# KhutornoyYaroslav/vcm-ts

Hardware: AMD Instinct MI355X
Metric: encoded frames/sec at 1920x1080 GOP-32 (higher is better)
Workload: dtype f32 (fp16x3 split-MFMA, fp32 accumulate)

## Files before the change

include/dcvc_hip.h:

```cpp
#ifndef DCVC_HIP_H
#define DCVC_HIP_H

#include <stdint.h>

#ifdef __cplusplus
extern "C" {
#endif

#define DCVC_OK 0
#define DCVC_E_ARG (-1)
#define DCVC_E_LAUNCH (-2)
#define DCVC_E_RANGE (-3)

#define DCVC_STATUS_ACT_SATURATED 1

#define DCVC_MAX_SEG 3

#define DCVC_PREC_FP32 0
#define DCVC_PREC_FP16X3 1

typedef struct {
    const float *ptr;
    int32_t C;
    int32_t cs;
} dcvc_seg;

typedef struct {
    dcvc_seg seg[DCVC_MAX_SEG];
    int32_t nseg;
    int32_t N, Hin, Win;
    int32_t in_act;
    float in_slope;
    const float *wpack;
    const float *bpack;
    int32_t ks;
    int32_t stride;
    int32_t Cout;
    int32_t Cout_pad;
    float *out;
    int32_t out_cs;
    int32_t out_act;
    float out_slope;
    int32_t pixel_shuffle;
    const float *res;
    int32_t res_cs;
    const float *res_gate;
    const float *res2;
    int32_t res2_cs;
    int32_t precision;
    int32_t *status;
    float *chan_partial;
    int32_t tile_row0;
    int32_t tile_rows;
    int32_t pair_taps;
} dcvc_conv_args;

int32_t dcvc_conv_tile_rows(int32_t ks, int32_t stride);

int32_t dcvc_conv_chan_partial_parts(int32_t ks, int32_t stride, int32_t Hout, int32_t Wout);
int dcvc_channel_mean_finish(const float *chan_partial, int32_t parts, int32_t row_stride, float *mean, int32_t N,
                             int32_t C, int32_t HW, void *stream);

int64_t dcvc_conv_pack_size(int32_t Cout, int32_t ks, int32_t nseg, const int32_t *seg_C, int32_t *cout_pad);

int dcvc_conv_pack_weights(const float *w, const float *b, int32_t Cout, int32_t ks, int32_t nseg,
                           const int32_t *seg_C, int32_t pixel_shuffle, int32_t precision, float *wpack,
                           float *bpack);

int64_t dcvc_conv_pack_size_paired(int32_t Cout, int32_t Cin, int32_t *cout_pad);
int dcvc_conv_pack_weights_paired(const float *w, const float *b, int32_t Cout, int32_t Cin, float *wpack, float *bpack);

int dcvc_conv2d(const dcvc_conv_args *a, void *stream);

int64_t dcvc_conv_small_pack_bytes(int32_t Cout, int32_t ks, int32_t nseg, const int32_t *seg_C);
int dcvc_conv_small_pack_weights(const float *w, const float *b, int32_t Cout, int32_t ks, int32_t nseg,
                                 const int32_t *seg_C, void *wpack, float *bpack);
int dcvc_conv2d_small(const dcvc_conv_args *a, void *stream);

int64_t dcvc_conv_k32_pack_bytes(int32_t Cout, int32_t ks, int32_t nseg, const int32_t *seg_C, int32_t *cout_pad);
int dcvc_conv_k32_pack_weights(const float *w, const float *b, int32_t Cout, int32_t ks, int32_t nseg,
                               const int32_t *seg_C, int32_t pixel_shuffle, void *wpack, float *bpack);
int dcvc_conv2d_k32(const dcvc_conv_args *a, void *stream);
int dcvc_conv_k32_set_waves(int32_t waves);

int dcvc_warp(const float *src, int32_t src_cs, const float *flow, int32_t flow_cs, float *out, int32_t out_cs,
              int32_t N, int32_t H, int32_t W, int32_t C, void *stream);
int dcvc_up2(const float *src, int32_t src_cs, float *out, int32_t out_cs, float *out2, int32_t out2_cs,
             int32_t N, int32_t H, int32_t W, int32_t C, float scale, void *stream);
int dcvc_down2(const float *src, int32_t src_cs, float *out, int32_t out_cs, int32_t N, int32_t H, int32_t W,
               int32_t C, float scale, int32_t avgpool_order, void *stream);
int dcvc_maxpool2(const float *src, int32_t src_cs, float *out, int32_t out_cs, int32_t N, int32_t H, int32_t W,
                  int32_t C, void *stream);
int dcvc_copy_channels(const float *src, int32_t src_cs, float *out, int32_t out_cs, int64_t npix, int32_t C,
                       void *stream);
int dcvc_nchw_to_nhwc(const float *src, float *out, int32_t out_cs, int32_t N, int32_t C, int32_t H, int32_t W,
                      void *stream);
int dcvc_nhwc_to_nchw(const float *src, int32_t src_cs, float *out, int32_t N, int32_t C, int32_t H, int32_t W,
                      int32_t clamp01, void *stream);

int dcvc_channel_mean(const float *src, int32_t src_cs, float *mean, float *scratch, int32_t N, int32_t HW,
                      int32_t C, void *stream);
int dcvc_se_gate(const float *mean, const float *w1, const float *w2, float *gate, int32_t N, int32_t C,
                 int32_t Cr, void *stream);

int dcvc_scale_channels(const float *src, int32_t src_cs, float *out, int32_t out_cs, const float *q_basic,
                        const float *q_scale, int32_t mode, int32_t N, int32_t HW, int32_t C, void *stream);
int dcvc_round_symbols(const float *z, int32_t z_cs, float *z_hat, int32_t zh_cs, int32_t *sym, int32_t N,
                       int32_t H, int32_t W, int32_t C, void *stream);
int dcvc_symbols_to_nhwc(const int32_t *sym, float *out, int32_t out_cs, int32_t N, int32_t H, int32_t W,
                         int32_t C, void *stream);

typedef struct {
    const float *y;
    int32_t y_cs;
    const float *fusion;
    int32_t fusion_cs;
    const float *spatial;
    int32_t spatial_cs;
    float *params;
    int32_t params_cs;
    float *y_hat;
    float *y_q;
    float *y_res;
    float *scales_hat;
    int32_t *sym;
    int32_t *idx;
    float *out;
    int32_t out_cs;
    const float *q_basic;
    const float *q_scale;
    int32_t N, H, W, C;
    int32_t step;
    const float *idx_edges;
    const float *forced_q;
} dcvc_dual_prior_args;

int dcvc_scale_indexes(const float *scales, int32_t *idx, int64_t n, const float *idx_edges, void *stream);

int dcvc_dual_prior_enc(const dcvc_dual_prior_args *a, void *stream);
int dcvc_dual_prior_dec_index(const dcvc_dual_prior_args *a, void *stream);
int dcvc_dual_prior_dec_apply(const dcvc_dual_prior_args *a, void *stream);

int dcvc_scale_bits(const float *y_q, const float *scales_hat, float *out, float *scratch, int32_t kind, int32_t N,
                    int64_t per_sample, void *stream);
int dcvc_factorized_bits(const float *z_hat, int32_t z_cs, const float *params, float *out, float *scratch, int32_t N,
                         int32_t HW, int32_t C, void *stream);
int dcvc_sq_err(const float *a, int32_t a_cs, const float *b, int32_t b_cs, float *out, float *scratch, int32_t N,
                int32_t HW, int32_t C, void *stream);

int32_t dcvc_cdf_table_cols(void);
int dcvc_build_scale_cdfs(const float *scales, int32_t n_scales, int32_t kind, int32_t *cdf, int32_t *sizes,
                          int32_t *offsets, void *stream);
int dcvc_build_factorized_cdfs(const float *params, int32_t C, int32_t *cdf, int32_t *sizes, int32_t *offsets, void *stream);

const char *dcvc_hip_version(void);

#ifdef __cplusplus
}
#endif
#endif
```

vcm_ts_amd/csrc/conv_mfma.hip:

```cpp
#include <hip/hip_runtime.h>
#include <stdint.h>
#include <stdlib.h>
#include <string.h>
#include <vector>

#include "dcvc_hip.h"
#include "kernel_common.h"

namespace {

constexpr int LDK = 20;


struct ConvK {
    const float *seg_ptr[DCVC_MAX_SEG];
    int seg_C[DCVC_MAX_SEG];
    int seg_cs[DCVC_MAX_SEG];
    int nseg;
    int Hin, Win, Hout, Wout;
    int in_act;
    float in_slope;
    const float *wpack;
    const float *bpack;
    int Cout, Cout_pad;
    float *out;
    int out_cs;
    int out_act;
    float out_slope;
    int ps;
    const float *res;
    int res_cs;
    const float *res_gate;
    const float *res2;
    int res2_cs;
    int vec_epi;
    int *status;
    float *chan_partial;
    int ntx;
    int ty0, nty;
    int band_rows;
};

inline long dev_env_long(const char *name, long dflt) {
    const char *dev = getenv("DCVC_DEV");
    if (!dev || strcmp(dev, "1") != 0) return dflt;
    const char *v = getenv(name);
    return v ? atol(v) : dflt;
}


template <int KS, int S, int RPW, int NT, bool SPLIT, bool PAIR = false>
__global__ __launch_bounds__(256, 2) void conv_mfma(const ConvK a) {
    static_assert(!PAIR || (KS == 7 && S == 1 && SPLIT), "tap pairing is built for the 7x7 split-fp16 layers");
    constexpr int BH = 4 * RPW, BW = 32, BN = 32 * NT;
    constexpr int PH = (BH - 1) * S + KS, PW = (BW - 1) * S + KS, PAD = KS / 2;
    constexpr int T = PAIR ? KS * 4 : KS * KS;
    constexpr int TPS = PAIR ? 4 : (KS == 3 && S == 1) ? 9 : KS;
    constexpr int NST = T / TPS;
    constexpr int EPI_LD = BN + 4;
    constexpr int LDS_MAIN = PH * PW * LDK + TPS * 4 * BN * 4, LDS_EPI = 4 * 32 * EPI_LD, LDS_RED = 4 * BN;
    __shared__ __attribute__((aligned(16))) float lds[LDS_MAIN > LDS_EPI + LDS_RED ? LDS_MAIN : LDS_EPI + LDS_RED];
    float *patch = lds;
    float *wl = lds + PH * PW * LDK;

    const int tid = threadIdx.x, lane = tid & 63, wave = tid >> 6;
    const int nbn = a.Cout_pad / BN;
    const int nb = blockIdx.x % nbn, tx = blockIdx.x / nbn;
    if (tx >= a.ntx) return;
    const int ty = blockIdx.y + a.ty0;
    const int x0 = tx * BW, y0 = ty * BH, n0 = nb * BN, img = blockIdx.z;

    f32x16 acc[RPW][NT];
#pragma unroll
    for (int m = 0; m < RPW; ++m)
#pragma unroll
        for (int n = 0; n < NT; ++n)
#pragma unroll
            for (int r = 0; r < 16; ++r) acc[m][n][r] = 0.f;

    const int a_base = ((wave * RPW * S) * PW + (lane & 31) * S) * LDK + (lane >> 5) * 4;
    const int b_base = ((lane >> 5) * BN + (lane & 31)) * 4;

    constexpr int NP = (PH * PW * 4 + 255) / 256, NW = (TPS * 4 * BN + 255) / 256;
    f32x4 rp[NP], rw[NW];
    struct Cursor {
        int s, c0, cg, st;
    };
    auto advance = [&](Cursor &k) {
        if (++k.st == NST) {
            k.st = 0;
            ++k.cg;
            k.c0 += MFMA_KC;
            if (k.c0 >= a.seg_C[k.s]) {
                ++k.s;
                k.c0 = 0;
            }
        }
    };
    int poff[NP];
    unsigned inpic = 0;
#pragma unroll
    for (int u = 0; u < NP; ++u) {
        const int i = tid + u * 256;
        const int p = i >> 2;
        const int py = p / PW, px = p - py * PW + (PAIR ? (i & 3) >> 1 : 0);
        const int gy = y0 * S - PAD + py, gx = x0 * S - PAD + px;
        const bool ok = i < PH * PW * 4 && gy >= 0 && gy < a.Hin && gx >= 0 && gx < a.Win;
        poff[u] = ok ? gy * a.Win + gx : 0;
        inpic |= (ok ? 1u : 0u) << u;
    }
    auto load_patch = [&](const Cursor &k) {
        const int C = a.seg_C[k.s], cs = a.seg_cs[k.s];
        const float *sp = a.seg_ptr[k.s] + (size_t)img * a.Hin * a.Win * cs;
        const int c = PAIR ? (tid & 1) * 4 : k.c0 + (tid & 3) * 4;
        const int cc = c < C ? c : 0;
#pragma unroll
        for (int u = 0; u < NP; ++u) rp[u] = *(const f32x4 *)(sp + (size_t)poff[u] * cs + cc);
    };
    auto store_patch = [&](const Cursor &k) {
        const int C = a.seg_C[k.s];
#pragma unroll
        for (int u = 0; u < NP; ++u) {
            const int i = tid + u * 256;
            if (i < PH * PW * 4) {
                const int c = PAIR ? (i & 1) * 4 : k.c0 + (i & 3) * 4;
                f32x4 v = ((inpic >> u) & 1u) && c < C ? rp[u] : (f32x4){0.f, 0.f, 0.f, 0.f};
                if (c + 3 >= C) {
                    if (c + 1 >= C) v[1] = 0.f;
                    if (c + 2 >= C) v[2] = 0.f;
                    v[3] = 0.f;
                }
                if (a.in_act) {
                    v[0] = act(v[0], a.in_slope);
                    v[1] = act(v[1], a.in_slope);
                    v[2] = act(v[2], a.in_slope);
                    v[3] = act(v[3], a.in_slope);
                }
                if (!SPLIT) {
                    *(f32x4 *)&patch[(i >> 2) * LDK + (i & 3) * 4] = v;
                } else {
                    f32x4 sv = v * ACT_SCALE;
#pragma unroll
                    for (int e = 0; e < 4; ++e) sv[e] = __builtin_amdgcn_fmed3f(sv[e], -F16_MAX, F16_MAX);
                    const f16x4 hi = __builtin_convertvector(sv, f16x4);
                    const f16x4 lo = __builtin_convertvector(sv - __builtin_convertvector(hi, f32x4), f16x4);
                    _Float16 *rec = (_Float16 *)&patch[(i >> 2) * LDK];
                    *(f16x4 *)&rec[(i & 3) * 4] = hi;
                    *(f16x4 *)&rec[16 + (i & 3) * 4] = lo;
                }
            }
        }
    };
    auto load_w = [&](const Cursor &k) {
        const float *wsrc = a.wpack + ((size_t)(k.cg * T + k.st * TPS) * 4) * a.Cout_pad * 4 + (size_t)n0 * 4;
#pragma unroll
        for (int u = 0; u < NW; ++u) {
            const int i = tid + u * 256;
            const int row = i / BN, col = i - row * BN;
            if (i < TPS * 4 * BN) rw[u] = *(const f32x4 *)(wsrc + ((size_t)row * a.Cout_pad + col) * 4);
        }
    };
    auto store_w = [&]() {
#pragma unroll
        for (int u = 0; u < NW; ++u) {
            const int i = tid + u * 256;
            if (i < TPS * 4 * BN) *(f32x4 *)&wl[i * 4] = rw[u];
        }
    };

    Cursor cur = {0, 0, 0, 0};
    load_patch(cur);
    load_w(cur);
    while (cur.s < a.nseg) {
        __syncthreads();
        if (cur.st == 0) store_patch(cur);
        store_w();
        __syncthreads();
        Cursor nxt = cur;
        advance(nxt);
        if (nxt.s < a.nseg) {
            if (nxt.st == 0) load_patch(nxt);
            load_w(nxt);
        }
        const int a_st = (TPS == T) ? 0 : cur.st * PW * LDK;
#pragma unroll
        for (int tt = 0; tt < TPS; ++tt) {
            const int ky = (TPS == T) ? tt / KS : 0, kx = PAIR ? 2 * tt : (TPS == T) ? tt % KS : tt;
            if (!SPLIT) {
#pragma unroll
                for (int k2 = 0; k2 < 2; ++k2) {
                    f32x4 af[RPW], bf[NT];
#pragma unroll
                    for (int m = 0; m < RPW; ++m)
                        af[m] = *(const f32x4 *)&patch[a_base + a_st + ((m * S + ky) * PW + kx) * LDK + k2 * 8];
#pragma unroll
                    for (int n = 0; n < NT; ++n)
                        bf[n] = *(const f32x4 *)&wl[b_base + ((tt * 4 + k2 * 2) * BN + n * 32) * 4];
#pragma unroll
                    for (int j = 0; j < 4; ++j)
#pragma unroll
                        for (int m = 0; m < RPW; ++m)
// ... 144 lines not shown
            int dy = 0, dx = 0, cf = ch;
            if (a.ps) {
                const int sub = ch / Cq;
                cf = ch - sub * Cq;
                dy = sub >> 1;
                dx = sub & 1;
            }
            const float gate = a.res_gate ? a.res_gate[(size_t)img * Cfin + cf] : 1.f;
            float rv[16], rv2[16];
#pragma unroll
            for (int r = 0; r < 16; ++r) {
                const int ox = x0 + (r & 3) + 8 * (r >> 2) + 4 * hh;
                const size_t pix = a.ps ? ((size_t)(img * Ho + 2 * oy + dy) * Wo + 2 * ox + dx)
                                        : ((size_t)(img * Ho + oy) * Wo + ox);
                rv[r] = (a.res && ox < a.Wout) ? a.res[pix * a.res_cs + cf] : 0.f;
                rv2[r] = (a.res2 && ox < a.Wout) ? a.res2[pix * a.res2_cs + cf] : 0.f;
            }
#pragma unroll
            for (int r = 0; r < 16; ++r) {
                const int ox = x0 + (r & 3) + 8 * (r >> 2) + 4 * hh;
                if (ox >= a.Wout) continue;
                float v = acc[m][n][r] * inv_scale + bias;
                if (a.out_act == 1) v = act(v, a.out_slope);
                else if (a.out_act == 2) v = fminf(fmaxf(v, 0.f), 1.f);
                const size_t pix = a.ps ? ((size_t)(img * Ho + 2 * oy + dy) * Wo + 2 * ox + dx)
                                        : ((size_t)(img * Ho + oy) * Wo + ox);
                if (a.out_act == 3) {
                    const float mk = rv2[r] > 0.f ? 1.f : a.out_slope;
                    v = a.res ? __builtin_fmaf(v, mk, rv[r]) : v * mk;
                } else {
                    if (a.res) v = a.res_gate ? __builtin_fmaf(rv[r], gate, v) : v + rv[r];
                    if (a.res2) v = rv2[r] + v;
                }
                if (a.status) vmax = fmaxf(vmax, fabsf(v));
                a.out[pix * a.out_cs + cf] = v;
            }
        }
    }
    if (a.status && !(vmax <= ACT_LIMIT)) atomicOr(a.status, DCVC_STATUS_ACT_SATURATED);
}


template <int KS, int S, int RPW, int NT, bool PAIR = false>
int launch(ConvK &k, int N, hipStream_t st, int precision) {
    constexpr int BH = 4 * RPW, BN = 32 * NT;
    k.ntx = (k.Wout + 31) / 32;
    static const bool xcd_pad = dev_env_long("DCVC_XCD_PAD", 0) != 0;
    unsigned gx = (unsigned)(k.ntx * (k.Cout_pad / BN));
    if (xcd_pad && gx >= 8) gx = (gx + 7) & ~7u;
    k.nty = (k.Hout + BH - 1) / BH;
    if (k.ty0 < 0 || k.ty0 >= k.nty) return DCVC_E_ARG;
    const int rows = k.band_rows > 0 ? (k.band_rows < k.nty - k.ty0 ? k.band_rows : k.nty - k.ty0) : k.nty;
    dim3 grid(gx, (unsigned)rows, (unsigned)N);
    if (PAIR)
        hipLaunchKernelGGL((conv_mfma<KS, S, RPW, NT, true, PAIR>), grid, dim3(256), 0, st, k);
    else if (precision == DCVC_PREC_FP16X3)
        hipLaunchKernelGGL((conv_mfma<KS, S, RPW, NT, true>), grid, dim3(256), 0, st, k);
    else
        hipLaunchKernelGGL((conv_mfma<KS, S, RPW, NT, false>), grid, dim3(256), 0, st, k);
    RET_LAUNCH();
}

}

extern "C" int64_t dcvc_conv_pack_size(int32_t Cout, int32_t ks, int32_t nseg, const int32_t *seg_C, int32_t *cout_pad) {
    if (Cout <= 0 || nseg <= 0 || nseg > DCVC_MAX_SEG || (ks != 1 && ks != 3 && ks != 7)) return DCVC_E_ARG;
    int chunks = 0;
    for (int s = 0; s < nseg; ++s) chunks += (seg_C[s] + MFMA_KC - 1) / MFMA_KC;
    const int cp = round_up(Cout, 32);
    if (cout_pad) *cout_pad = cp;
    return (int64_t)chunks * ks * ks * 4 * cp * 4;
}

extern "C" int dcvc_conv_pack_weights(const float *w, const float *b, int32_t Cout, int32_t ks, int32_t nseg,
                                      const int32_t *seg_C, int32_t pixel_shuffle, int32_t precision, float *wpack,
                                      float *bpack) {
    if (precision != DCVC_PREC_FP32 && precision != DCVC_PREC_FP16X3) return DCVC_E_ARG;
    int32_t cp = 0;
    const int64_t total = dcvc_conv_pack_size(Cout, ks, nseg, seg_C, &cp);
    if (total < 0 || (pixel_shuffle && (Cout & 3))) return DCVC_E_ARG;
    const int T = ks * ks;
    int Cin = 0;
    for (int s = 0; s < nseg; ++s) Cin += seg_C[s];
    memset(wpack, 0, (size_t)total * sizeof(float));
    memset(bpack, 0, (size_t)cp * sizeof(float));
    const int Cq = Cout / 4;
    _Float16 *base = (_Float16 *)wpack;
    int cg = 0, cin0 = 0;
    for (int s = 0; s < nseg; ++s) {
        for (int c0 = 0; c0 < seg_C[s]; c0 += MFMA_KC, ++cg) {
            for (int t = 0; t < T; ++t)
                for (int cc = 0; cc < MFMA_KC && c0 + cc < seg_C[s]; ++cc)
                    for (int n = 0; n < Cout; ++n) {
                        const int np = pixel_shuffle ? ps_packed_channel(n, Cq) : n;
                        const float v = w[((size_t)n * Cin + cin0 + c0 + cc) * T + t];
                        if (precision == DCVC_PREC_FP32) {
                            wpack[mfma_wpack_f32(cg, T, t, cc, cp, np)] = v;
                        } else {
                            float sv = v * WGT_SCALE;
                            sv = sv > F16_MAX ? F16_MAX : (sv < -F16_MAX ? -F16_MAX : sv);
                            const SplitF16 p = split_f16(sv);
                            base[mfma_wpack_f16(cg, T, t, cc, cp, np, 0)] = p.hi;
                            base[mfma_wpack_f16(cg, T, t, cc, cp, np, 1)] = p.lo;
                        }
                    }
        }
        cin0 += seg_C[s];
    }
    for (int n = 0; n < Cout; ++n) bpack[pixel_shuffle ? ps_packed_channel(n, Cq) : n] = b ? b[n] : 0.f;
    return DCVC_OK;
}

extern "C" int64_t dcvc_conv_pack_size_paired(int32_t Cout, int32_t Cin, int32_t *cout_pad) {
    if (Cout <= 0 || Cin <= 0 || Cin > 8) return DCVC_E_ARG;
    const int cp = round_up(Cout, 32);
    if (cout_pad) *cout_pad = cp;
    return (int64_t)7 * 4 * 4 * cp * 4;
}

extern "C" int dcvc_conv_pack_weights_paired(const float *w, const float *b, int32_t Cout, int32_t Cin, float *wpack, float *bpack) {
    int32_t cp = 0;
    const int64_t total = dcvc_conv_pack_size_paired(Cout, Cin, &cp);
    if (total < 0 || !w || !wpack || !bpack) return DCVC_E_ARG;
    memset(wpack, 0, (size_t)total * sizeof(float));
    memset(bpack, 0, (size_t)cp * sizeof(float));
    _Float16 *base = (_Float16 *)wpack;
    bool clamped = false;
    for (int ky = 0; ky < 7; ++ky)
        for (int kx = 0; kx < 7; ++kx) {
            const int step = ky * 4 + (kx >> 1), h = kx & 1;
            for (int c = 0; c < Cin; ++c)
                for (int n = 0; n < Cout; ++n) {
                    float sv = w[((size_t)n * Cin + c) * 49 + ky * 7 + kx] * WGT_SCALE;
                    if (!(fabsf(sv) <= F16_MAX)) { clamped = true; sv = sv > 0.f ? F16_MAX : -F16_MAX; }
                    const SplitF16 p = split_f16(sv);
                    base[mfma_wpack_f16(0, 28, step, 8 * h + c, cp, n, 0)] = p.hi;
                    base[mfma_wpack_f16(0, 28, step, 8 * h + c, cp, n, 1)] = p.lo;
                }
        }
    for (int n = 0; n < Cout; ++n) bpack[n] = b ? b[n] : 0.f;
    return clamped ? DCVC_E_RANGE : DCVC_OK;
}

static int tile_rows(int ks, int stride) { return stride == 2 ? 4 : 8; }

extern "C" int32_t dcvc_conv_tile_rows(int32_t ks, int32_t stride) { return tile_rows(ks, stride); }

extern "C" int32_t dcvc_conv_chan_partial_parts(int32_t ks, int32_t stride, int32_t Hout, int32_t Wout) {
    if (Hout <= 0 || Wout <= 0 || (stride != 1 && stride != 2)) return DCVC_E_ARG;
    const int bh = tile_rows(ks, stride);
    return ((Wout + 31) / 32) * ((Hout + bh - 1) / bh);
}

extern "C" int dcvc_conv2d(const dcvc_conv_args *a, void *stream) {
    if (!conv_args_ok(a)) return DCVC_E_ARG;
    if (a->stride != 1 && a->stride != 2) return DCVC_E_ARG;
    if (a->precision != DCVC_PREC_FP32 && a->precision != DCVC_PREC_FP16X3) return DCVC_E_ARG;
    if (a->Cout_pad % 32 || a->Cout > a->Cout_pad || (a->pixel_shuffle && (a->Cout & 3))) return DCVC_E_ARG;
    if (a->out_act < 0 || a->out_act > 3) return DCVC_E_ARG;
    if (a->out_act == 3 && (!a->res2 || a->res_gate || a->chan_partial || a->pixel_shuffle)) return DCVC_E_ARG;
    ConvK k;
    memset(&k, 0, sizeof(k));
    copy_conv_args_full(k, a);
    k.Hin = a->Hin;
    k.Win = a->Win;
    const int pad = a->ks / 2;
    k.Hout = (a->Hin + 2 * pad - a->ks) / a->stride + 1;
    k.Wout = (a->Win + 2 * pad - a->ks) / a->stride + 1;
    k.vec_epi = vec_epilogue_ok(a);
    if (a->chan_partial && (!k.vec_epi || a->pixel_shuffle)) return DCVC_E_ARG;
    hipStream_t st = (hipStream_t)stream;
    const bool wide = (a->Cout_pad % 64) == 0;
    const int key = a->ks * 10 + a->stride;
    if (a->stride == 1 && !a->pair_taps && !a->chan_partial && a->tile_rows <= 0) {
        const long wgs8 = (long)((k.Wout + 31) / 32) * ((k.Hout + 7) / 8) * (a->Cout_pad / (wide ? 64 : 32)) * a->N;
        static const long rows4_below = dev_env_long("DCVC_ROWS4_WGS", 384);
        if (wgs8 < rows4_below) {
            if (a->ks == 3) return wide ? launch<3, 1, 1, 2>(k, a->N, st, a->precision) : launch<3, 1, 1, 1>(k, a->N, st, a->precision);
            if (a->ks == 7) return wide ? launch<7, 1, 1, 2>(k, a->N, st, a->precision) : launch<7, 1, 1, 1>(k, a->N, st, a->precision);
            if (a->ks == 1) return wide ? launch<1, 1, 1, 2>(k, a->N, st, a->precision) : launch<1, 1, 1, 1>(k, a->N, st, a->precision);
        }
    }
    switch (key) {
        case 11: return wide ? launch<1, 1, 2, 2>(k, a->N, st, a->precision) : launch<1, 1, 2, 1>(k, a->N, st, a->precision);
        case 12: return wide ? launch<1, 2, 1, 2>(k, a->N, st, a->precision) : launch<1, 2, 1, 1>(k, a->N, st, a->precision);
        case 31:
            return wide ? launch<3, 1, 2, 2>(k, a->N, st, a->precision) : launch<3, 1, 2, 1>(k, a->N, st, a->precision);
        case 32: return wide ? launch<3, 2, 1, 2>(k, a->N, st, a->precision) : launch<3, 2, 1, 1>(k, a->N, st, a->precision);
        case 71:
            if (a->pair_taps) {
                if (a->nseg != 1 || a->seg[0].C > 8 || a->precision != DCVC_PREC_FP16X3 || a->pixel_shuffle) return DCVC_E_ARG;
                return wide ? launch<7, 1, 2, 2, true>(k, a->N, st, a->precision) : launch<7, 1, 2, 1, true>(k, a->N, st, a->precision);
            }
            return wide ? launch<7, 1, 2, 2>(k, a->N, st, a->precision) : launch<7, 1, 2, 1>(k, a->N, st, a->precision);
        default: return DCVC_E_ARG;
    }
}
```

vcm_ts_amd/csrc/conv_small.hip:

```cpp
#include <hip/hip_runtime.h>
#include <stdint.h>
#include <string.h>

#include "dcvc_hip.h"
#include "kernel_common.h"

namespace {

constexpr int KC = 16;

struct SmallK {
    const float *seg_ptr[DCVC_MAX_SEG];
    int seg_C[DCVC_MAX_SEG];
    int seg_cs[DCVC_MAX_SEG];
    int nseg;
    int H, W;
    int in_act;
    float in_slope;
    const char *wpack;
    const float *bpack;
    int Cout;
    float *out;
    int out_cs, out_act;
    float out_slope;
    const float *res;
    int res_cs;
    int *status;
};

template <int KS>
__global__ __launch_bounds__(256, 3) void conv_small(const SmallK a) {
    constexpr int RPW = 2, BH = 4 * RPW, BW = 32, PAD = KS / 2, PH = BH + KS - 1, PW = BW + KS - 1, T = KS * KS;
    constexpr int TPS = KS, NST = KS;
    constexpr int PATCH_F = PH * PW * 16;
    constexpr int SLAB_F = TPS * 4 * 16 * 4;
    __shared__ __attribute__((aligned(16))) float lds[PATCH_F + SLAB_F];
    char *patch = (char *)lds;
    float *wl = lds + PATCH_F;

    const int tid = threadIdx.x, lane = tid & 63, wave = tid >> 6;
    const int x0 = blockIdx.x * BW, y0 = blockIdx.y * BH, img = blockIdx.z;
    const int pr = lane & 15, g = lane >> 4;

    f32x4 acc[RPW][2];
#pragma unroll
    for (int m = 0; m < RPW; ++m)
#pragma unroll
        for (int hf = 0; hf < 2; ++hf) acc[m][hf] = (f32x4){0.f, 0.f, 0.f, 0.f};

    constexpr int NP = (PH * PW * 4 + 255) / 256, NW = (SLAB_F / 4 + 255) / 256;
    f32x4 rp[NP], rw[NW];
    struct Cursor {
        int s, c0, cg, st;
    };
    auto advance = [&](Cursor &k) {
        if (++k.st == NST) {
            k.st = 0;
            ++k.cg;
            k.c0 += KC;
            if (k.c0 >= a.seg_C[k.s]) {
                ++k.s;
                k.c0 = 0;
            }
        }
    };
    int poff[NP];
    unsigned inpic = 0;
#pragma unroll
    for (int u = 0; u < NP; ++u) {
        const int i = tid + u * 256;
        const int p = i >> 2;
        const int py = p / PW, px = p - py * PW;
        const int gy = y0 - PAD + py, gx = x0 - PAD + px;
        const bool ok = i < PH * PW * 4 && gy >= 0 && gy < a.H && gx >= 0 && gx < a.W;
        poff[u] = ok ? gy * a.W + gx : 0;
        inpic |= (ok ? 1u : 0u) << u;
    }
    auto load_patch = [&](const Cursor &k) {
        const int C = a.seg_C[k.s], cs = a.seg_cs[k.s];
        const float *sp = a.seg_ptr[k.s] + (size_t)img * a.H * a.W * cs;
        const int c = k.c0 + (tid & 3) * 4;
        const int cc = c < C ? c : 0;
#pragma unroll
        for (int u = 0; u < NP; ++u) rp[u] = *(const f32x4 *)(sp + (size_t)poff[u] * cs + cc);
    };
    auto store_patch = [&](const Cursor &k) {
        const int C = a.seg_C[k.s];
#pragma unroll
        for (int u = 0; u < NP; ++u) {
            const int i = tid + u * 256;
            if (i < PH * PW * 4) {
                const int qd = i & 3, p = i >> 2;
                const int c = k.c0 + qd * 4;
                f32x4 v = ((inpic >> u) & 1u) && c < C ? rp[u] : (f32x4){0.f, 0.f, 0.f, 0.f};
                if (c + 3 >= C) {
                    if (c + 1 >= C) v[1] = 0.f;
                    if (c + 2 >= C) v[2] = 0.f;
                    v[3] = 0.f;
                }
                if (a.in_act) {
#pragma unroll
                    for (int e = 0; e < 4; ++e) v[e] = act(v[e], a.in_slope);
                }
                f32x4 sv = v * ACT_SCALE;
#pragma unroll
                for (int e = 0; e < 4; ++e) sv[e] = __builtin_amdgcn_fmed3f(sv[e], -F16_MAX, F16_MAX);
                const f16x4 hi = __builtin_convertvector(sv, f16x4);
                const f16x4 lo = __builtin_convertvector(sv - __builtin_convertvector(hi, f32x4), f16x4);
                const int sw = (p >> 1) & 3, h = qd >> 1;
                char *rec = patch + p * 64 + (qd & 1) * 8;
                *(f16x4 *)(rec + ((h ^ sw) << 4)) = hi;
                *(f16x4 *)(rec + (((2 + h) ^ sw) << 4)) = lo;
            }
        }
    };
    auto load_w = [&](const Cursor &k) {
        const f32x4 *wsrc = (const f32x4 *)(a.wpack + ((size_t)(k.cg * T + k.st * TPS)) * 1024);
#pragma unroll
        for (int u = 0; u < NW; ++u) {
            const int i = tid + u * 256;
            if (i < SLAB_F / 4) rw[u] = wsrc[i];
        }
    };
    auto store_w = [&]() {
#pragma unroll
        for (int u = 0; u < NW; ++u) {
            const int i = tid + u * 256;
            if (i < SLAB_F / 4) *(f32x4 *)&wl[i * 4] = rw[u];
        }
    };

    Cursor cur = {0, 0, 0, 0};
    load_patch(cur);
    load_w(cur);
    const f16x8 zero8 = {0, 0, 0, 0, 0, 0, 0, 0};
    while (cur.s < a.nseg) {
        __syncthreads();
        if (cur.st == 0) store_patch(cur);
        store_w();
        __syncthreads();
        Cursor nxt = cur;
        advance(nxt);
        if (nxt.s < a.nseg) {
            if (nxt.st == 0) load_patch(nxt);
            load_w(nxt);
        }
#pragma unroll
        for (int tt = 0; tt < TPS; ++tt) {
            const f16x8 b1 = *(const f16x8 *)&wl[((tt * 4 + (g & 1)) * 16 + pr) * 4];
            const f16x8 b2 = g < 2 ? *(const f16x8 *)&wl[((tt * 4 + 2 + g) * 16 + pr) * 4] : zero8;
#pragma unroll
            for (int m = 0; m < RPW; ++m)
#pragma unroll
                for (int hf = 0; hf < 2; ++hf) {
                    const int p = (wave * RPW + m + cur.st) * PW + hf * 16 + pr + tt;
                    const f16x8 av = *(const f16x8 *)(patch + p * 64 + ((g ^ ((p >> 1) & 3)) << 4));
                    acc[m][hf] = __builtin_amdgcn_mfma_f32_16x16x32_f16(av, b1, acc[m][hf], 0, 0, 0);
                    acc[m][hf] = __builtin_amdgcn_mfma_f32_16x16x32_f16(av, b2, acc[m][hf], 0, 0, 0);
                }
        }
        cur = nxt;
    }

    const float inv_scale = 1.f / (ACT_SCALE * WGT_SCALE);
    const int ch = pr;
    bool sat = false;
    if (ch < a.Cout) {
        const float bias = a.bpack[ch];
#pragma unroll
        for (int m = 0; m < RPW; ++m) {
            const int oy = y0 + wave * RPW + m;
            if (oy >= a.H) continue;
            float rv[2][4];
#pragma unroll
            for (int hf = 0; hf < 2; ++hf)
#pragma unroll
                for (int j = 0; j < 4; ++j) {
                    const int ox = x0 + hf * 16 + g * 4 + j;
                    rv[hf][j] = (a.res && ox < a.W) ? a.res[((size_t)(img * a.H + oy) * a.W + ox) * a.res_cs + ch] : 0.f;
                }
#pragma unroll
            for (int hf = 0; hf < 2; ++hf)
#pragma unroll
                for (int j = 0; j < 4; ++j) {
                    const int ox = x0 + hf * 16 + g * 4 + j;
                    if (ox >= a.W) continue;
                    float v = acc[m][hf][j] * inv_scale + bias;
                    if (a.out_act == 1) v = act(v, a.out_slope);
                    else if (a.out_act == 2) v = fminf(fmaxf(v, 0.f), 1.f);
                    if (a.res) v += rv[hf][j];
                    if (a.status && !(fabsf(v) <= ACT_LIMIT)) sat = true;
                    a.out[((size_t)(img * a.H + oy) * a.W + ox) * a.out_cs + ch] = v;
                }
        }
    }
    if (sat) atomicOr(a.status, DCVC_STATUS_ACT_SATURATED);
}

}

extern "C" int64_t dcvc_conv_small_pack_bytes(int32_t Cout, int32_t ks, int32_t nseg, const int32_t *seg_C) {
    if (Cout <= 0 || Cout > 16 || nseg <= 0 || nseg > DCVC_MAX_SEG || (ks != 3 && ks != 7)) return DCVC_E_ARG;
    int chunks = 0;
    for (int s = 0; s < nseg; ++s) {
        if (seg_C[s] <= 0) return DCVC_E_ARG;
        chunks += (seg_C[s] + KC - 1) / KC;
    }
    return (int64_t)chunks * ks * ks * 1024;
}

extern "C" int dcvc_conv_small_pack_weights(const float *w, const float *b, int32_t Cout, int32_t ks, int32_t nseg,
                                            const int32_t *seg_C, void *wpack, float *bpack) {
    const int64_t total = dcvc_conv_small_pack_bytes(Cout, ks, nseg, seg_C);
    if (total < 0 || !w || !wpack || !bpack) return DCVC_E_ARG;
    const int T = ks * ks;
    int Cin = 0;
    for (int s = 0; s < nseg; ++s) Cin += seg_C[s];
    memset(wpack, 0, (size_t)total);
    for (int n = 0; n < 16; ++n) bpack[n] = (b && n < Cout) ? b[n] : 0.f;
    _Float16 *base = (_Float16 *)wpack;
    int status = DCVC_OK, cg = 0, cin0 = 0;
    for (int s = 0; s < nseg; ++s) {
        for (int c0 = 0; c0 < seg_C[s]; c0 += KC, ++cg)
            for (int t = 0; t < T; ++t)
                for (int cc = 0; cc < KC && c0 + cc < seg_C[s]; ++cc)
                    for (int n = 0; n < Cout; ++n) {
                        float sv = w[((size_t)n * Cin + cin0 + c0 + cc) * T + t] * WGT_SCALE;
                        if (!(fabsf(sv) <= F16_MAX)) { status = DCVC_E_RANGE; sv = sv > 0.f ? F16_MAX : -F16_MAX; }
                        const SplitF16 p = split_f16(sv);
                        const size_t blk = ((size_t)cg * T + t) * 4;
                        base[((blk + (cc >> 3)) * 16 + n) * 8 + (cc & 7)] = p.hi;
                        base[((blk + 2 + (cc >> 3)) * 16 + n) * 8 + (cc & 7)] = p.lo;
                    }
        cin0 += seg_C[s];
    }
    return status;
}

extern "C" int dcvc_conv2d_small(const dcvc_conv_args *a, void *stream) {
    if (!conv_args_ok(a)) return DCVC_E_ARG;
    if (a->out_act < 0 || a->out_act > 2) return DCVC_E_ARG;
    if (a->tile_rows > 0) return DCVC_E_ARG;
    if (a->Cout <= 0 || a->Cout > 16 || (a->ks != 3 && a->ks != 7) || a->stride != 1 || a->pixel_shuffle || a->res_gate ||
        a->res2 || a->chan_partial || a->precision != DCVC_PREC_FP16X3 || a->N <= 0)
        return DCVC_E_ARG;
    SmallK k;
    memset(&k, 0, sizeof(k));
    copy_conv_args(k, a);
    k.H = a->Hin, k.W = a->Win;
    dim3 grid((unsigned)((a->Win + 31) / 32), (unsigned)((a->Hin + 7) / 8), (unsigned)a->N);
    if (a->ks == 7)
        hipLaunchKernelGGL(conv_small<7>, grid, dim3(256), 0, (hipStream_t)stream, k);
    else
        hipLaunchKernelGGL(conv_small<3>, grid, dim3(256), 0, (hipStream_t)stream, k);
    RET_LAUNCH();
}
```

vcm_ts_amd/lib.py:

```python
from __future__ import annotations

import ctypes as C
import os

HERE = os.path.dirname(os.path.abspath(__file__))
CSRC = os.path.join(HERE, "csrc")


class LibraryMissing(RuntimeError):
    pass


class KernelError(RuntimeError):
    pass


def _load(name):
    path = os.environ.get("DCVC_HIP_LIB") if name == "libdcvc_hip.so" and os.environ.get("DCVC_HIP_LIB") else \
        os.path.join(CSRC, name)
    if not os.path.exists(path):
        raise LibraryMissing(f"{path} not built; run `make -C {CSRC}` (no CPU fallback exists)")
    return C.CDLL(path)


# ... 32 lines not shown
        ("seg", Seg * 3), ("nseg", C.c_int32), ("N", C.c_int32), ("Hin", C.c_int32), ("Win", C.c_int32),
        ("in_act", C.c_int32), ("in_slope", C.c_float), ("wpack", C.c_void_p), ("bpack", C.c_void_p),
        ("ks", C.c_int32), ("stride", C.c_int32), ("Cout", C.c_int32), ("Cout_pad", C.c_int32),
        ("out", C.c_void_p), ("out_cs", C.c_int32), ("out_act", C.c_int32), ("out_slope", C.c_float),
        ("pixel_shuffle", C.c_int32), ("res", C.c_void_p), ("res_cs", C.c_int32), ("res_gate", C.c_void_p),
        ("res2", C.c_void_p), ("res2_cs", C.c_int32), ("precision", C.c_int32), ("status", C.c_void_p),
        ("chan_partial", C.c_void_p), ("tile_row0", C.c_int32), ("tile_rows", C.c_int32), ("pair_taps", C.c_int32),
    ]


class DualPriorArgs(C.Structure):
    _fields_ = [
        ("y", C.c_void_p), ("y_cs", C.c_int32), ("fusion", C.c_void_p), ("fusion_cs", C.c_int32),
        ("spatial", C.c_void_p), ("spatial_cs", C.c_int32), ("params", C.c_void_p), ("params_cs", C.c_int32),
        ("y_hat", C.c_void_p), ("y_q", C.c_void_p), ("y_res", C.c_void_p), ("scales_hat", C.c_void_p),
        ("sym", C.c_void_p), ("idx", C.c_void_p), ("out", C.c_void_p), ("out_cs", C.c_int32),
        ("q_basic", C.c_void_p), ("q_scale", C.c_void_p), ("N", C.c_int32), ("H", C.c_int32), ("W", C.c_int32),
        ("C", C.c_int32), ("step", C.c_int32), ("idx_edges", C.c_void_p), ("forced_q", C.c_void_p),
    ]


class ConvBwdArgs(C.Structure):
    _fields_ = [
        ("dout", C.c_void_p), ("dout_cs", C.c_int32), ("out", C.c_void_p), ("out_cs", C.c_int32),
        ("res", C.c_void_p), ("res_cs", C.c_int32), ("gate", C.c_void_p), ("res2", C.c_void_p), ("res2_cs", C.c_int32),
        ("dres", C.c_void_p), ("dres_cs", C.c_int32), ("dres2", C.c_void_p), ("dres2_cs", C.c_int32),
        ("dpre", C.c_void_p), ("dpre_cs", C.c_int32), ("zs", C.c_int32), ("Hd", C.c_int32), ("Wd", C.c_int32),
        ("N", C.c_int32), ("Ho", C.c_int32), ("Wo", C.c_int32), ("Cout", C.c_int32), ("pixel_shuffle", C.c_int32),
        ("act", C.c_int32), ("slope", C.c_float),
    ]


class WgradArgs(C.Structure):
    _fields_ = [
        ("x", C.c_void_p), ("x_cs", C.c_int32), ("C", C.c_int32), ("in_act", C.c_int32), ("in_slope", C.c_float),
        ("dpre", C.c_void_p), ("dpre_cs", C.c_int32), ("zs", C.c_int32), ("Hd", C.c_int32), ("Wd", C.c_int32),
        ("N", C.c_int32), ("Hin", C.c_int32), ("Win", C.c_int32), ("Ho", C.c_int32), ("Wo", C.c_int32),
        ("Cout", C.c_int32), ("ks", C.c_int32), ("stride", C.c_int32), ("dw", C.c_void_p), ("Cin_total", C.c_int32),
        ("cin_offset", C.c_int32), ("scratch", C.c_void_p), ("scratch_floats", C.c_int64), ("overwrite", C.c_int32),
        ("db", C.c_void_p), ("precision", C.c_int32),
    ]


class PackJob(C.Structure):
    _fields_ = [
        ("w", C.c_void_p), ("b", C.c_void_p), ("Cout", C.c_int32), ("Cin_total", C.c_int32), ("ks", C.c_int32),
        ("nseg", C.c_int32), ("seg_C", C.c_int32 * 3), ("cin_offset", C.c_int32), ("pixel_shuffle", C.c_int32),
        ("precision", C.c_int32), ("transposed", C.c_int32), ("wpack", C.c_void_p), ("bpack", C.c_void_p),
    ]


class DualPriorBwdArgs(C.Structure):
    _fields_ = [
        ("y", C.c_void_p), ("y_cs", C.c_int32), ("fusion", C.c_void_p), ("fusion_cs", C.c_int32),
        ("y_hat", C.c_void_p), ("dout", C.c_void_p), ("dout_cs", C.c_int32), ("dy_res", C.c_void_p),
        ("dscales_hat", C.c_void_p), ("dparams", C.c_void_p), ("dparams_cs", C.c_int32),
        ("dspatial", C.c_void_p), ("dspatial_cs", C.c_int32), ("dy", C.c_void_p), ("dy_cs", C.c_int32),
        ("dfusion", C.c_void_p), ("dfusion_cs", C.c_int32), ("dq_plane", C.c_void_p),
        ("q_basic", C.c_void_p), ("q_scale", C.c_void_p), ("N", C.c_int32), ("H", C.c_int32), ("W", C.c_int32),
        ("C", C.c_int32), ("step", C.c_int32),
    ]


class ColorCoeffs(C.Structure):
    _fields_ = [(n, C.c_float) for n in ("y_off", "c_off", "y_scale", "c_scale", "crr", "cgb", "cgr", "cbb", "kr", "kg", "kb",
                                         "icb", "icr", "y_range", "c_range")] + \
               [(n, C.c_int32) for n in ("max_code", "bit_depth", "siting", "matrix", "range")]


class RoiBox(C.Structure):
    _fields_ = [(n, C.c_int32) for n in ("x1", "y1", "x2", "y2", "cls")]


class RoiClassRec(C.Structure):
    _fields_ = [("border", C.c_int32), ("shrink", C.c_int32), ("feather", C.c_float * 64)]


PRECISIONS = {"fp32": 0, "fp16x3": 1}

_hip = None
i32, i64, f32, vp = C.c_int32, C.c_int64, C.c_float, C.c_void_p

_SIGS = {
    "dcvc_conv2d": [C.POINTER(ConvArgs), vp],
    "dcvc_conv_pack_weights": [vp, vp, i32, i32, i32, vp, i32, i32, vp, vp],
    "dcvc_conv_pack_weights_paired": [vp, vp, i32, i32, vp, vp],
    "dcvc_conv2d_small": [C.POINTER(ConvArgs), vp],
    "dcvc_conv_small_pack_weights": [vp, vp, i32, i32, i32, vp, vp, vp],
    "dcvc_conv2d_k32": [C.POINTER(ConvArgs), vp],
    "dcvc_conv_k32_pack_weights": [vp, vp, i32, i32, i32, vp, i32, vp, vp],
    "dcvc_conv_k32_set_waves": [i32],
    "dcvc_warp": [vp, i32, vp, i32, vp, i32, i32, i32, i32, i32, vp],
    "dcvc_up2": [vp, i32, vp, i32, vp, i32, i32, i32, i32, i32, f32, vp],
    "dcvc_down2": [vp, i32, vp, i32, i32, i32, i32, i32, f32, i32, vp],
    "dcvc_maxpool2": [vp, i32, vp, i32, i32, i32, i32, i32, vp],
    "dcvc_copy_channels": [vp, i32, vp, i32, i64, i32, vp],
    "dcvc_nchw_to_nhwc": [vp, vp, i32, i32, i32, i32, i32, vp],
    "dcvc_nhwc_to_nchw": [vp, i32, vp, i32, i32, i32, i32, i32, vp],
    "dcvc_channel_mean": [vp, i32, vp, vp, i32, i32, i32, vp],
    "dcvc_se_gate": [vp, vp, vp, vp, i32, i32, i32, vp],
    "dcvc_channel_mean_finish": [vp, i32, i32, vp, i32, i32, i32, vp],
    "dcvc_scale_channels": [vp, i32, vp, i32, vp, vp, i32, i32, i32, i32, vp],
    "dcvc_round_symbols": [vp, i32, vp, i32, vp, i32, i32, i32, i32, vp],
    "dcvc_symbols_to_nhwc": [vp, vp, i32, i32, i32, i32, i32, vp],
    "dcvc_scale_indexes": [vp, vp, i64, vp, vp],
    "dcvc_dual_prior_enc": [C.POINTER(DualPriorArgs), vp],
    "dcvc_dual_prior_dec_index": [C.POINTER(DualPriorArgs), vp],
    "dcvc_dual_prior_dec_apply": [C.POINTER(DualPriorArgs), vp],
    "dcvc_build_scale_cdfs": [vp, i32, i32, vp, vp, vp, vp],
    "dcvc_build_factorized_cdfs": [vp, i32, vp, vp, vp, vp],
    "dcvc_scale_bits": [vp, vp, vp, vp, i32, i32, i64, vp],
    "dcvc_factorized_bits": [vp, i32, vp, vp, vp, i32, i32, i32, vp],
    "dcvc_sq_err": [vp, i32, vp, i32, vp, vp, i32, i32, i32, vp],
    "dcvc_conv_pack_weights_dev": [vp, vp, i32, i32, i32, i32, vp, i32, i32, i32, i32, vp, vp, vp],
    "dcvc_pack_plan_create": [C.POINTER(PackJob), i32, C.POINTER(C.c_void_p)],
    "dcvc_pack_plan_run": [vp, vp],
    "dcvc_pack_plan_destroy": [vp],
    "dcvc_conv_bwd_prologue": [C.POINTER(ConvBwdArgs), vp],
    "dcvc_conv_wgrad": [C.POINTER(WgradArgs), vp],
    "dcvc_channel_dot": [vp, i32, vp, i32, vp, vp, i32, i32, i32, i32, i32, vp],
    "dcvc_mask_accumulate": [vp, i32, vp, i32, f32, vp, i32, i64, i32, vp],
    "dcvc_add_planes": [vp, i32, vp, i32, vp, i32, i64, i32, vp],
    "dcvc_warp_bwd": [vp, i32, vp, i32, vp, i32, vp, i32, vp, i32, i32, i32, i32, i32, vp, vp],
    "dcvc_up2_bwd": [vp, i32, vp, i32, i32, i32, i32, i32, f32, vp],
    "dcvc_down2_bwd": [vp, i32, vp, i32, i32, i32, i32, i32, f32, vp],
    "dcvc_maxpool2_bwd": [vp, i32, vp, i32, vp, i32, i32, i32, i32, i32, vp],
    "dcvc_se_bwd": [vp, vp, vp, vp, vp, vp, vp, vp, i32, i32, i32, vp],
    "dcvc_add_channel_vec": [vp, i32, vp, f32, i32, i32, i32, vp],
    "dcvc_scale_channels_bwd": [vp, i32, vp, i32, vp, vp, i32, i32, i32, i32, vp],
    "dcvc_q_finish": [vp, vp, vp, vp, vp, vp, i32, i32, vp],
    "dcvc_dual_prior_bwd": [C.POINTER(DualPriorBwdArgs), vp],
    "dcvc_scale_bits_bwd": [vp, vp, vp, vp, vp, i32, i32, i64, vp],
    "dcvc_factorized_bits_bwd": [vp, i32, vp, vp, vp, i32, vp, i32, i32, i32, vp],
    "dcvc_sq_err_bwd": [vp, i32, vp, i32, vp, vp, i32, i32, i32, i32, vp],
    "dcvc_drans_encode": [vp, vp, i32, i32, i64, vp, i32, i32, vp, vp, i32, vp, i64, vp, i64, vp, vp, vp, vp],
    "dcvc_drans_decode": [vp, i64, vp, vp, vp, i32, i32, i64, vp, i32, i32, vp, vp, vp, i32, vp, vp, vp],
    "dcvc_drans_build_lut": [vp, i32, i32, vp, vp],
    "dcvc_ms_ssim": [vp, vp, i32, i32, i32, i32, i32, i64, i32, i64, f32, i32, vp, vp, vp, vp, vp],
    "dcvc_ms_ssim_grad": [vp, vp, i32, i32, i32, i32, i32, i64, i32, i64, f32, i32, vp, vp, vp, vp],
    "dcvc_color_coeffs": [i32, i32, i32, i32, vp],
    "dcvc_yuv420_to_rgb": [vp, vp, vp, i32, i32, i32, i32, vp, vp, i32, i32, i32, i64, i32, vp],
    "dcvc_rgb_to_yuv420": [vp, i32, i32, i32, i64, vp, vp, vp, vp, i32, i32, vp, vp, vp, i32, i32, vp, vp],
    "dcvc_roi_residual": [vp, i32, i64, vp, i32, i64, i32, i32, vp, vp, i32, vp, i64, i64, i32, i32, i32, i32, vp],
    "dcvc_roi_fuse": [vp, i32, i64, vp, i64, i64, i32, i32, i32, i32, i32, i32, vp, vp, i32, vp, i32, vp, i32, i64, vp],
    "dcvc_roi_sse": [vp, i32, i64, vp, i32, i64, i32, i32, vp, vp, i32, vp, i32, vp, vp],
    "dcvc_scene_hist": [vp, i32, i64, i32, i32, vp, vp],
}

METRICS_SYMBOLS = ["dcvc_ms_ssim", "dcvc_ms_ssim_grad", "dcvc_ms_ssim_workspace_bytes"]
COLOR_SYMBOLS = ["dcvc_color_coeffs", "dcvc_yuv420_to_rgb", "dcvc_rgb_to_yuv420"]
ROI_SYMBOLS = ["dcvc_roi_residual", "dcvc_roi_fuse", "dcvc_roi_sse"]
SCENE_SYMBOLS = ["dcvc_scene_hist"]
HIP_SYMBOLS = sorted([s for s in _SIGS if s not in METRICS_SYMBOLS + COLOR_SYMBOLS + ROI_SYMBOLS + SCENE_SYMBOLS] +
                     ["dcvc_cdf_table_cols", "dcvc_conv_pack_size", "dcvc_conv_pack_size_paired", "dcvc_conv_small_pack_bytes", "dcvc_conv_k32_pack_bytes", "dcvc_conv_tile_rows", "dcvc_conv_chan_partial_parts", "dcvc_hip_version", "dcvc_conv_wgrad_scratch_min",
                      "dcvc_drans_default_lanes", "dcvc_drans_scratch_words"])
RANS_SYMBOLS = [
    "dcvc_rans_encoder_create", "dcvc_rans_encoder_destroy", "dcvc_rans_encoder_reset",
    "dcvc_rans_encoder_encode_with_indexes", "dcvc_rans_encoder_flush_bound", "dcvc_rans_encoder_flush",
    "dcvc_rans_decoder_create", "dcvc_rans_decoder_destroy", "dcvc_rans_decoder_set_stream",
    "dcvc_rans_decoder_decode_stream", "dcvc_pmf_to_quantized_cdf",
]


def hip():
    global _hip
    if _hip is None:
        L = _load("libdcvc_hip.so")
        for name, sig in _SIGS.items():
            fn = getattr(L, name)
            fn.argtypes = sig
            fn.restype = C.c_int
        L.dcvc_pack_plan_destroy.restype = None
        L.dcvc_conv_pack_size.argtypes = [i32, i32, i32, vp, C.POINTER(i32)]
        L.dcvc_conv_pack_size.restype = i64
        L.dcvc_conv_pack_size_paired.argtypes = [i32, i32, C.POINTER(i32)]
        L.dcvc_conv_pack_size_paired.restype = i64
        L.dcvc_cdf_table_cols.argtypes = []
        L.dcvc_cdf_table_cols.restype = i32
        L.dcvc_conv_chan_partial_parts.argtypes = [i32, i32, i32, i32]
        L.dcvc_conv_chan_partial_parts.restype = i32
        L.dcvc_conv_small_pack_bytes.argtypes = [i32, i32, i32, vp]
        L.dcvc_conv_small_pack_bytes.restype = i64
        L.dcvc_conv_tile_rows.argtypes = [i32, i32]
        L.dcvc_conv_tile_rows.restype = i32
        L.dcvc_conv_k32_pack_bytes.argtypes = [i32, i32, i32, vp, C.POINTER(i32)]
        L.dcvc_conv_k32_pack_bytes.restype = i64
        L.dcvc_hip_version.restype = C.c_char_p
        L.dcvc_conv_wgrad_scratch_min.argtypes = [i32, i32, i32]
        L.dcvc_conv_wgrad_scratch_min.restype = i64
        L.dcvc_drans_default_lanes.argtypes = [i64]
        L.dcvc_drans_default_lanes.restype = i32
        L.dcvc_drans_scratch_words.argtypes = [i64, i32]
        L.dcvc_drans_scratch_words.restype = i64
        L.dcvc_ms_ssim_workspace_bytes.argtypes = [i32, i32, i32, i32, i32]
        L.dcvc_ms_ssim_workspace_bytes.restype = i64
        _hip = L
    return _hip


def check(code, what):
    if code != 0:
        raise KernelError(f"{what} failed with status {code}")
```

Before: 40.85.

## Add 16-row tiles for 7x7 Cout32 convs and two-row weight stages in conv_small

Adds a 'tall' path for 7x7 stride-1 convolutions with 32 padded output channels. When the grid is large enough, these launch with four rows per wave (16-row tiles), so the input patch halo is reused across more output rows. A runtime setter and an env threshold control the choice. Separately, conv_small for KS=7 now stages two filter rows of weights per pipeline step instead of one, which cuts the number of stage/sync iterations. The cost is more LDS, more registers, and a guarded tail stage.

```diff
diff --git a/include/dcvc_hip.h b/include/dcvc_hip.h
--- a/include/dcvc_hip.h
+++ b/include/dcvc_hip.h
@@ -71,6 +71,10 @@
 int dcvc_conv_pack_weights_paired(const float *w, const float *b, int32_t Cout, int32_t Cin, float *wpack, float *bpack);
 
 int dcvc_conv2d(const dcvc_conv_args *a, void *stream);
+#define DCVC_ROWS16_AUTO 0
+#define DCVC_ROWS16_ALWAYS 1
+#define DCVC_ROWS16_NEVER 2
+int dcvc_conv_set_rows16(int32_t mode);
 
 int64_t dcvc_conv_small_pack_bytes(int32_t Cout, int32_t ks, int32_t nseg, const int32_t *seg_C);
 int dcvc_conv_small_pack_weights(const float *w, const float *b, int32_t Cout, int32_t ks, int32_t nseg,
diff --git a/vcm_ts_amd/csrc/conv_mfma.hip b/vcm_ts_amd/csrc/conv_mfma.hip
--- a/vcm_ts_amd/csrc/conv_mfma.hip
+++ b/vcm_ts_amd/csrc/conv_mfma.hip
@@ -47,6 +47,8 @@
     const char *v = getenv(name);
     return v ? atol(v) : dflt;
 }
+
+int g_rows16 = DCVC_ROWS16_AUTO;
 
 
 template <int KS, int S, int RPW, int NT, bool SPLIT, bool PAIR = false>
@@ -497,6 +499,12 @@
     return ((Wout + 31) / 32) * ((Hout + bh - 1) / bh);
 }
 
+extern "C" int dcvc_conv_set_rows16(int32_t mode) {
+    if (mode != DCVC_ROWS16_AUTO && mode != DCVC_ROWS16_ALWAYS && mode != DCVC_ROWS16_NEVER) return DCVC_E_ARG;
+    g_rows16 = mode;
+    return DCVC_OK;
+}
+
 extern "C" int dcvc_conv2d(const dcvc_conv_args *a, void *stream) {
     if (!conv_args_ok(a)) return DCVC_E_ARG;
     if (a->stride != 1 && a->stride != 2) return DCVC_E_ARG;
@@ -517,10 +525,16 @@
     hipStream_t st = (hipStream_t)stream;
     const bool wide = (a->Cout_pad % 64) == 0;
     const int key = a->ks * 10 + a->stride;
+    bool tall = false;
+    if (a->ks == 7 && a->stride == 1 && a->Cout_pad == 32 && !a->chan_partial && a->tile_rows <= 0 && g_rows16 != DCVC_ROWS16_NEVER) {
+        const long wgs16 = (long)((k.Wout + 31) / 32) * ((k.Hout + 15) / 16) * a->N;
+        static const long rows16_from = dev_env_long("DCVC_ROWS16_WGS", 512);
+        tall = g_rows16 == DCVC_ROWS16_ALWAYS || wgs16 >= rows16_from;
+    }
     if (a->stride == 1 && !a->pair_taps && !a->chan_partial && a->tile_rows <= 0) {
         const long wgs8 = (long)((k.Wout + 31) / 32) * ((k.Hout + 7) / 8) * (a->Cout_pad / (wide ? 64 : 32)) * a->N;
         static const long rows4_below = dev_env_long("DCVC_ROWS4_WGS", 384);
-        if (wgs8 < rows4_below) {
+        if (!tall && wgs8 < rows4_below) {
             if (a->ks == 3) return wide ? launch<3, 1, 1, 2>(k, a->N, st, a->precision) : launch<3, 1, 1, 1>(k, a->N, st, a->precision);
             if (a->ks == 7) return wide ? launch<7, 1, 1, 2>(k, a->N, st, a->precision) : launch<7, 1, 1, 1>(k, a->N, st, a->precision);
             if (a->ks == 1) return wide ? launch<1, 1, 1, 2>(k, a->N, st, a->precision) : launch<1, 1, 1, 1>(k, a->N, st, a->precision);
@@ -535,8 +549,10 @@
         case 71:
             if (a->pair_taps) {
                 if (a->nseg != 1 || a->seg[0].C > 8 || a->precision != DCVC_PREC_FP16X3 || a->pixel_shuffle) return DCVC_E_ARG;
+                if (tall) return launch<7, 1, 4, 1, true>(k, a->N, st, a->precision);
                 return wide ? launch<7, 1, 2, 2, true>(k, a->N, st, a->precision) : launch<7, 1, 2, 1, true>(k, a->N, st, a->precision);
             }
+            if (tall) return launch<7, 1, 4, 1>(k, a->N, st, a->precision);
             return wide ? launch<7, 1, 2, 2>(k, a->N, st, a->precision) : launch<7, 1, 2, 1>(k, a->N, st, a->precision);
         default: return DCVC_E_ARG;
     }
diff --git a/vcm_ts_amd/csrc/conv_small.hip b/vcm_ts_amd/csrc/conv_small.hip
--- a/vcm_ts_amd/csrc/conv_small.hip
+++ b/vcm_ts_amd/csrc/conv_small.hip
@@ -31,7 +31,9 @@
 template <int KS>
 __global__ __launch_bounds__(256, 3) void conv_small(const SmallK a) {
     constexpr int RPW = 2, BH = 4 * RPW, BW = 32, PAD = KS / 2, PH = BH + KS - 1, PW = BW + KS - 1, T = KS * KS;
-    constexpr int TPS = KS, NST = KS;
+    constexpr int RPS = KS == 7 ? 2 : KS;
+    constexpr int TPS = RPS * KS, NST = (KS + RPS - 1) / RPS;
+    constexpr int ROW_UNROLL = KS == 7 ? 1 : RPS;
     constexpr int PATCH_F = PH * PW * 16;
     constexpr int SLAB_F = TPS * 4 * 16 * 4;
     __shared__ __attribute__((aligned(16))) float lds[PATCH_F + SLAB_F];
@@ -119,7 +121,7 @@
 #pragma unroll
         for (int u = 0; u < NW; ++u) {
             const int i = tid + u * 256;
-            if (i < SLAB_F / 4) rw[u] = wsrc[i];
+            if (i < SLAB_F / 4 && k.st * TPS * 64 + i < T * 64) rw[u] = wsrc[i];
         }
     };
     auto store_w = [&]() {
@@ -145,19 +147,24 @@
             if (nxt.st == 0) load_patch(nxt);
             load_w(nxt);
         }
-#pragma unroll
-        for (int tt = 0; tt < TPS; ++tt) {
-            const f16x8 b1 = *(const f16x8 *)&wl[((tt * 4 + (g & 1)) * 16 + pr) * 4];
-            const f16x8 b2 = g < 2 ? *(const f16x8 *)&wl[((tt * 4 + 2 + g) * 16 + pr) * 4] : zero8;
-#pragma unroll
-            for (int m = 0; m < RPW; ++m)
-#pragma unroll
-                for (int hf = 0; hf < 2; ++hf) {
-                    const int p = (wave * RPW + m + cur.st) * PW + hf * 16 + pr + tt;
-                    const f16x8 av = *(const f16x8 *)(patch + p * 64 + ((g ^ ((p >> 1) & 3)) << 4));
-                    acc[m][hf] = __builtin_amdgcn_mfma_f32_16x16x32_f16(av, b1, acc[m][hf], 0, 0, 0);
-                    acc[m][hf] = __builtin_amdgcn_mfma_f32_16x16x32_f16(av, b2, acc[m][hf], 0, 0, 0);
-                }
+#pragma unroll ROW_UNROLL
+        for (int r = 0; r < RPS; ++r) {
+            if (KS % RPS != 0 && cur.st * RPS + r >= KS) break;
+#pragma unroll
+            for (int kx = 0; kx < KS; ++kx) {
+                const int tt = r * KS + kx;
+                const f16x8 b1 = *(const f16x8 *)&wl[((tt * 4 + (g & 1)) * 16 + pr) * 4];
+                const f16x8 b2 = g < 2 ? *(const f16x8 *)&wl[((tt * 4 + 2 + g) * 16 + pr) * 4] : zero8;
+#pragma unroll
+                for (int m = 0; m < RPW; ++m)
+#pragma unroll
+                    for (int hf = 0; hf < 2; ++hf) {
+                        const int p = (wave * RPW + m + cur.st * RPS + r) * PW + hf * 16 + pr + kx;
+                        const f16x8 av = *(const f16x8 *)(patch + p * 64 + ((g ^ ((p >> 1) & 3)) << 4));
+                        acc[m][hf] = __builtin_amdgcn_mfma_f32_16x16x32_f16(av, b1, acc[m][hf], 0, 0, 0);
+                        acc[m][hf] = __builtin_amdgcn_mfma_f32_16x16x32_f16(av, b2, acc[m][hf], 0, 0, 0);
+                    }
+            }
         }
         cur = nxt;
     }
diff --git a/vcm_ts_amd/lib.py b/vcm_ts_amd/lib.py
--- a/vcm_ts_amd/lib.py
+++ b/vcm_ts_amd/lib.py
@@ -208,7 +208,7 @@
 ROI_SYMBOLS = ["dcvc_roi_residual", "dcvc_roi_fuse", "dcvc_roi_sse"]
 SCENE_SYMBOLS = ["dcvc_scene_hist"]
 HIP_SYMBOLS = sorted([s for s in _SIGS if s not in METRICS_SYMBOLS + COLOR_SYMBOLS + ROI_SYMBOLS + SCENE_SYMBOLS] +
-                     ["dcvc_cdf_table_cols", "dcvc_conv_pack_size", "dcvc_conv_pack_size_paired", "dcvc_conv_small_pack_bytes", "dcvc_conv_k32_pack_bytes", "dcvc_conv_tile_rows", "dcvc_conv_chan_partial_parts", "dcvc_hip_version", "dcvc_conv_wgrad_scratch_min",
+                     ["dcvc_cdf_table_cols", "dcvc_conv_pack_size", "dcvc_conv_pack_size_paired", "dcvc_conv_small_pack_bytes", "dcvc_conv_k32_pack_bytes", "dcvc_conv_tile_rows", "dcvc_conv_chan_partial_parts", "dcvc_conv_set_rows16", "dcvc_hip_version", "dcvc_conv_wgrad_scratch_min",
                       "dcvc_drans_default_lanes", "dcvc_drans_scratch_words"])
 RANS_SYMBOLS = [
     "dcvc_rans_encoder_create", "dcvc_rans_encoder_destroy", "dcvc_rans_encoder_reset",
@@ -239,6 +239,8 @@
         L.dcvc_conv_small_pack_bytes.restype = i64
         L.dcvc_conv_tile_rows.argtypes = [i32, i32]
         L.dcvc_conv_tile_rows.restype = i32
+        L.dcvc_conv_set_rows16.argtypes = [i32]
+        L.dcvc_conv_set_rows16.restype = C.c_int
         L.dcvc_conv_k32_pack_bytes.argtypes = [i32, i32, i32, vp, C.POINTER(i32)]
         L.dcvc_conv_k32_pack_bytes.restype = i64
         L.dcvc_hip_version.restype = C.c_char_p
```

Result: no change. 41.10, median of 6 (+0.6%).
